# peteroh23/ModulationDetectionCNN

Measured on AMD Instinct MI355X. Metric: I/Q frames/sec (2x128, VT-CNN2, batch=2^20), higher is better.
Workload: dtype bf16; 1 GPU; vtcnn2-c11-bf16-n2^20; topology=vtcnn2, classes=11, frames_per_gpu=1048576, global_batch=1048576, parallelism=batch-shard x1 (no collective), outputs=softmax probabilities f32 + argmax int32, frames_per_forward_call=1048576, full=False

## Files before the change

modulationdetectioncnn_amd/csrc/mdc_api.hip:

```cpp
#include "mdc_internal.h"

#include <cstdlib>
#include <cstring>
#include <exception>
#include <mutex>
#include <new>

namespace mdc {

static thread_local char g_err[512] = "";

void set_error(const char* fmt, ...) {
    va_list ap;
    va_start(ap, fmt);
    vsnprintf(g_err, sizeof(g_err), fmt, ap);
    va_end(ap);
}

int upload(mdc_model* m, int idx, const void* host, size_t bytes) {
    if (m->d_pack[idx]) {
        (void)hipFree(m->d_pack[idx]);
        m->d_pack[idx] = nullptr;
    }
    MDC_HIP(hipMalloc(&m->d_pack[idx], bytes));
// ... 28 lines not shown
    if (hop < 1 || hop > (int64_t)1 << 24) { set_error("%s: hop must be in 1..2^24 sample pairs (got %lld)", who, (long long)hop); return MDC_EINVAL; }
    if (!(level > 0.f) || !(level <= 3.402823466e38f)) { set_error("%s: level must be finite and > 0", who); return MDC_EINVAL; }
    if ((flags & ~MDC_IQ_REMOVE_DC) != 0) { set_error("%s: unknown flag bits 0x%x", who, flags & ~MDC_IQ_REMOVE_DC); return MDC_EINVAL; }
    return MDC_OK;
}

}

using namespace mdc;

static int layer_layout(mdc_model* m) {
    const mdc_topology& t = m->topo;
    switch (t.kind) {
        case MDC_KIND_DEPLOYED:
            if (t.filters != 3 && t.filters != 10) { set_error("deployed: filters must be 3 or 10 (got %d)", t.filters); return MDC_ENOTSUP; }
            if (t.classes != 3) { set_error("deployed: classes must be 3 (got %d)", t.classes); return MDC_ENOTSUP; }
            m->nlayers = 2;
            m->nk[0] = 2 * (size_t)t.filters;            m->nb[0] = t.filters;
            m->nk[1] = 258 * (size_t)t.filters * t.classes; m->nb[1] = t.classes;
            m->slots = {{"mdc_deployed_fwd"}};
            return MDC_OK;
        case MDC_KIND_VTCNN2:
            if (t.classes < 2 || t.classes > 16) { set_error("vtcnn2: classes must be in 2..16 (got %d)", t.classes); return MDC_ENOTSUP; }
            m->nlayers = 4;
            m->nk[0] = (size_t)kC1 * 3;               m->nb[0] = kC1;
            m->nk[1] = (size_t)kC2 * kC1 * 2 * 3;     m->nb[1] = kC2;
            m->nk[2] = (size_t)kFeat * kHid;          m->nb[2] = kHid;
            m->nk[3] = (size_t)kHid * t.classes;      m->nb[3] = t.classes;
            m->slots = {{"mdc_vt_conv"}, {"mdc_vt_dense1"}, {"mdc_vt_head"}};
            return MDC_OK;
        case MDC_KIND_CNNPY:
            if (t.filters < 1 || t.filters > 10 || t.hidden < 1 || t.hidden > 16 || t.classes < 2 || t.classes > 16) {
                set_error("cnnpy: need filters 1..10, hidden 1..16, classes 2..16 (got %d,%d,%d)", t.filters, t.hidden, t.classes);
                return MDC_ENOTSUP;
            }
            m->nlayers = 3;
            m->nk[0] = 2 * 128 * (size_t)t.filters;        m->nb[0] = t.filters;
            m->nk[1] = 3 * (size_t)t.filters * t.hidden;    m->nb[1] = t.hidden;
            m->nk[2] = (size_t)t.hidden * t.classes;        m->nb[2] = t.classes;
            m->slots = {{"mdc_dense_chain"}};
            return MDC_OK;
        default:
            set_error("unknown topology kind %d", t.kind);
            return MDC_EINVAL;
    }
}

extern "C" {

int mdc_abi_version(void) { return MDC_ABI_VERSION; }

const char* mdc_last_error(void) { return g_err; }

int mdc_create(const mdc_topology* topo, int device, mdc_model** out) {
    return guarded("mdc_create", [&]() -> int {
        if (!topo || !out) { set_error("mdc_create: null argument"); return MDC_EINVAL; }
        *out = nullptr;
        if ((topo->reserved[0] & ~MDC_OPT_ALL) != 0) { set_error("mdc_create: unknown option bits 0x%x in reserved[0]", topo->reserved[0]); return MDC_EINVAL; }
        for (int i = 1; i < 4; ++i) if (topo->reserved[i] != 0) { set_error("mdc_create: reserved[1..3] must be 0"); return MDC_EINVAL; }
        if ((topo->reserved[0] & MDC_OPT_FP8_BF16_FEATURES) && topo->kind != MDC_KIND_VTCNN2) {
            set_error("mdc_create: MDC_OPT_FP8_BF16_FEATURES applies to MDC_KIND_VTCNN2 only");
            return MDC_EINVAL;
        }
        int ndev = 0;
        if (hipGetDeviceCount(&ndev) != hipSuccess || ndev == 0) { set_error("no HIP device available"); return MDC_ENODEV; }
        if (device < 0 || device >= ndev) { set_error("device %d out of range (have %d)", device, ndev); return MDC_ENODEV; }
        hipDeviceProp_t prop;
        MDC_HIP(hipGetDeviceProperties(&prop, device));
        if (std::strncmp(prop.gcnArchName, "gfx950", 6) != 0) {
            set_error("device %d is %s; libmdc.so carries gfx950 (MI355X) code only", device, prop.gcnArchName);
            return MDC_ENODEV;
        }
        mdc_model* m = new (std::nothrow) mdc_model();
        if (!m) { set_error("out of host memory"); return MDC_ENOMEM; }
        m->topo = *topo;
        m->device = device;
#ifdef MDC_ALTERNATES
        {
            auto flag = [](const char* name, int when) { const char* e = getenv(name); return e && atoi(e) == when; };
            if (flag("MDC_CONV_SCHED", 0)) m->alt |= kAltConvHipcc;
            if (flag("MDC_DENSE1_PHASED", 0)) m->alt |= kAltDense1Simple;
            if (flag("MDC_DEP_F32_MFMA", 1)) m->alt |= kAltDepF32Mfma;
            if (flag("MDC_D1_FUSED_HEAD", 0)) m->alt |= kAltSeparateHead;
            if (const char* e = getenv("MDC_DEP_RING")) m->alt_ring = atoi(e);
        }
#endif
        int rc = MDC_ENOMEM;
        try { rc = layer_layout(m); } catch (...) { delete m; throw; }
        if (rc != MDC_OK) { delete m; return rc; }
        *out = m;
        return MDC_OK;
    });
}

int mdc_num_layers(const mdc_model* m) {
    if (!m) { set_error("null model"); return MDC_EINVAL; }
    return m->nlayers;
}

int mdc_layer_sizes(const mdc_model* m, int layer, size_t* kernel_elems, size_t* bias_elems) {
    if (!m || layer < 0 || layer >= m->nlayers) { set_error("mdc_layer_sizes: bad layer %d", layer); return MDC_EINVAL; }
    if (kernel_elems) *kernel_elems = m->nk[layer];
    if (bias_elems) *bias_elems = m->nb[layer];
    return MDC_OK;
}

int mdc_set_weights(mdc_model* m, int layer, const float* kernel_host, size_t kernel_elems,
                    const float* bias_host, size_t bias_elems) {
    return guarded("mdc_set_weights", [&]() -> int {
        if (!m || !kernel_host || !bias_host) { set_error("mdc_set_weights: null argument"); return MDC_EINVAL; }
        if (m->finalized) { set_error("mdc_set_weights: model is finalized (immutable)"); return MDC_ESTATE; }
        if (layer < 0 || layer >= m->nlayers) { set_error("mdc_set_weights: layer %d out of range 0..%d", layer, m->nlayers - 1); return MDC_EINVAL; }
        if (kernel_elems != m->nk[layer] || bias_elems != m->nb[layer]) {
            set_error("mdc_set_weights: layer %d expects kernel %zu / bias %zu elements, got %zu / %zu",
                      layer, m->nk[layer], m->nb[layer], kernel_elems, bias_elems);
            return MDC_EINVAL;
        }
        m->have[layer] = false;
        m->hk[layer].assign(kernel_host, kernel_host + kernel_elems);
        m->hb[layer].assign(bias_host, bias_host + bias_elems);
        m->have[layer] = true;
        return MDC_OK;
    });
}

int mdc_finalize(mdc_model* m, int dtype) {
    return guarded("mdc_finalize", [&]() -> int {
        if (!m) { set_error("null model"); return MDC_EINVAL; }
        if (m->finalized) { set_error("mdc_finalize: already finalized"); return MDC_ESTATE; }
        for (int l = 0; l < m->nlayers; ++l)
            if (!m->have[l]) { set_error("mdc_finalize: layer %d has no weights", l); return MDC_ESTATE; }
        if (dtype != MDC_F32 && dtype != MDC_BF16 && dtype != MDC_FP8 && dtype != MDC_F16) { set_error("unknown dtype %d", dtype); return MDC_EINVAL; }
        if (dtype == MDC_F16 && m->topo.kind != MDC_KIND_DEPLOYED) { set_error("f16 is implemented for the deployed nets only"); return MDC_ENOTSUP; }
        if (dtype == MDC_FP8 && m->topo.kind == MDC_KIND_CNNPY) { set_error("fp8 is implemented for the vtcnn2 and deployed families only"); return MDC_ENOTSUP; }
        if ((m->topo.reserved[0] & MDC_OPT_FP8_BF16_FEATURES) && dtype != MDC_FP8) { set_error("mdc_finalize: MDC_OPT_FP8_BF16_FEATURES is an option of the MDC_FP8 mode"); return MDC_EINVAL; }
        if (dtype == MDC_BF16 && m->topo.kind == MDC_KIND_CNNPY) { set_error("bf16 is implemented for the vtcnn2 and deployed families only"); return MDC_ENOTSUP; }
        m->dtype = dtype;
        DeviceScope dev(m->device);
        if (!dev.ok) { set_error("mdc_finalize: cannot select device %d", m->device); return MDC_EIO; }
        int rc;
        switch (m->topo.kind) {
            case MDC_KIND_DEPLOYED:
                rc = deployed_pack(m);
                if (rc == MDC_OK) rc = deployed_q612_pack(m);
                if (rc == MDC_OK && dtype != MDC_F32) rc = deployed_bf16_pack(m);
                break;
            case MDC_KIND_VTCNN2:   rc = vtcnn2_pack(m); break;
            case MDC_KIND_CNNPY:    rc = cnnpy_pack(m); break;
            default: rc = MDC_EINVAL;
        }
        if (rc != MDC_OK) return rc;
        for (int l = 0; l < m->nlayers; ++l) {
            std::vector<float>().swap(m->hk[l]);
            std::vector<float>().swap(m->hb[l]);
        }
        m->finalized = true;
        return MDC_OK;
    });
}

size_t mdc_workspace_bytes(const mdc_model* m, int64_t n) {
    if (!m || n <= 0) return 0;
    if (m->topo.kind == MDC_KIND_VTCNN2) return vtcnn2_workspace_bytes(m, n);
    return 0;
}

// ... 273 lines not shown
```

modulationdetectioncnn_amd/csrc/mdc_internal.h:

```cpp
#pragma once
#include <hip/hip_runtime.h>
#include <cstdarg>
#include <cstdint>
#include <cstdio>
#include <exception>
#include <mutex>
#include <new>
#include <string>
#include <type_traits>
#include <vector>

#include "mdc.h"

namespace mdc {

void set_error(const char* fmt, ...);

template <class Fn>
inline int guarded(const char* what, Fn&& fn) noexcept {
    try {
        return fn();
    } catch (const std::bad_alloc&) {
        set_error("%s: out of host memory", what);
        return MDC_ENOMEM;
    } catch (const std::exception& e) {
        set_error("%s: %s", what, e.what());
        return MDC_EIO;
    } catch (...) {
        set_error("%s: unexpected exception", what);
        return MDC_EIO;
    }
}

#define MDC_HIP(call)                                                                      \
    do {                                                                                   \
        hipError_t e_ = (call);                                                            \
        if (e_ != hipSuccess) {                                                            \
            mdc::set_error("%s failed: %s (%s:%d)", #call, hipGetErrorString(e_), __FILE__, __LINE__); \
            return MDC_EIO;                                                                \
        }                                                                                  \
    } while (0)

constexpr int kRows = 2;
constexpr int kSamples = 128;
constexpr int kFrameFloats = kRows * kSamples;

constexpr int kC1 = 256;
constexpr int kW1 = 130;
constexpr int kC2 = 80;
constexpr int kW2 = 132;
constexpr int kFeat = kC2 * kW2;
constexpr int kHid = 256;

__host__ __device__ constexpr int feat16_index(int w, int o) {
    return (w >> 1) * (2 * kC2) + (o < 64 ? (w & 1) * 64 + o : 128 + 2 * (o - 64) + (w & 1));
}

__host__ __device__ constexpr int feat8_index(int w, int o) {
    return (w >> 2) * (4 * kC2) + (o < 64 ? ((w >> 1) & 1) * 128 + 8 * (o >> 2) + 4 * (w & 1) + (o & 3) : 256 + 4 * (o - 64) + (w & 3));
}

__device__ __forceinline__ uint2 load8_unaligned(const unsigned char* p) {
    uint2 r;
    __builtin_memcpy(&r, p, 8);
    return r;
}

struct NfArgs {
    unsigned char* flags;
    unsigned long long* count;
    int poison;
};
template <bool CHECK> using HopOrNf = typename std::conditional<CHECK, NfArgs, long>::type;
__device__ __forceinline__ long hop_of(long h) { return h; }
__device__ __forceinline__ long hop_of(const NfArgs&) { return 256; }
__device__ __forceinline__ NfArgs nf_of(long) { return NfArgs{nullptr, nullptr, 0}; }
__device__ __forceinline__ NfArgs nf_of(const NfArgs& a) { return a; }
constexpr unsigned kNfInfBits = 0x7F800000u;
__device__ __forceinline__ unsigned nf_absbits_max4(const float4 v) {
    return max(max(__float_as_uint(v.x) & 0x7FFFFFFFu, __float_as_uint(v.y) & 0x7FFFFFFFu),
               max(__float_as_uint(v.z) & 0x7FFFFFFFu, __float_as_uint(v.w) & 0x7FFFFFFFu));
}

enum { kAltConvHipcc = 1,
       kAltDense1Simple = 2,
       kAltDepF32Mfma = 4,
       kAltSeparateHead = 8 };

struct ProfSlot {
    const char* name;
    std::vector<hipEvent_t> ev;
    double total_ms = 0;
    int64_t launches = 0;
};

}

struct mdc_model {
    mdc_topology topo{};
    int device = 0;
    int dtype = MDC_F32;
    bool finalized = false;
    int nlayers = 0;
    size_t nk[4]{}, nb[4]{};
    std::vector<float> hk[4], hb[4];
    bool have[4]{};

    void* d_pack[8]{};
    size_t pack_bytes[8]{};

    int alt = 0;
    int alt_ring = -1;
    float fp8_input_absmax = 0.02f;
    float fp8_feature_absmax = 0.f;
    int fp8_feat_scale_log2 = 0;
    bool fp8_e4m3_features = false;
    float fp8_feat_divisor = 1.f;
    int feat_scale_log2 = 0;

    bool profiling = false;
    std::vector<mdc::ProfSlot> slots;
    std::mutex prof_mu;

    void* host_ctx = nullptr;
    std::mutex host_mu;
};

namespace mdc {

struct ProfScope {
    mdc_model* m;
    int slot;
    hipStream_t s;
    hipEvent_t start = nullptr;
    ProfScope(const mdc_model* mm, int slot_, hipStream_t s_);
    ~ProfScope();
    ProfScope(const ProfScope&) = delete;
    ProfScope& operator=(const ProfScope&) = delete;
};

int upload(mdc_model* m, int idx, const void* host, size_t bytes);

struct DeviceScope {
    int prev = -1, want;
    bool ok = true;
    explicit DeviceScope(int device) : want(device) {
        if (hipGetDevice(&prev) != hipSuccess) prev = -1;
        if (prev != want && hipSetDevice(want) != hipSuccess) ok = false;
    }
    ~DeviceScope() { if (prev >= 0 && prev != want) (void)hipSetDevice(prev); }
    DeviceScope(const DeviceScope&) = delete;
    DeviceScope& operator=(const DeviceScope&) = delete;
};

int predict_host(mdc_model* m, const float* x_host, int64_t n, float* probs_host, int32_t* labels_host, int64_t chunk_frames);
int predict_host_checked(mdc_model* m, const float* x_host, int64_t n, float* probs_host, int32_t* labels_host, uint8_t* nonfinite_host,
                         int64_t* nonfinite_count, int policy, int64_t chunk_frames);
int predict_host_iq_u8(mdc_model* m, const uint8_t* iq_host, int64_t n, int64_t hop, float scale, float* probs_host, int32_t* labels_host,
                       int64_t chunk_frames);
int predict_host_iq_u8_norm(mdc_model* m, const uint8_t* iq_host, int64_t n, int64_t hop, float level, int flags, float* probs_host,
                            int32_t* labels_host, mdc_iq_window_stats* stats_host, int64_t chunk_frames);
int predict_host_iq(mdc_model* m, const void* iq_host, int format, int64_t n, int64_t hop, float scale, float* probs_host, int32_t* labels_host,
                    int64_t chunk_frames);
int predict_host_iq_norm(mdc_model* m, const void* iq_host, int format, int64_t n, int64_t hop, float level, int flags, float* probs_host,
                         int32_t* labels_host, mdc_iq_window_stats64* stats_host, int64_t chunk_frames);
void host_ctx_free(mdc_model* m);

int deployed_pack(mdc_model* m);
int deployed_f32m_pack(mdc_model* m);
int deployed_f32m_forward(const mdc_model* m, const float* x, int64_t n, float* probs, int32_t* labels, float* tap_dense, hipStream_t s);
// ... 42 lines not shown
```

modulationdetectioncnn_amd/csrc/vtcnn2_bf16_dense1.hip:

```cpp
#include "vtcnn2_bf16_common.h"
#include "dense_chain_common.h"

#include <cstdlib>

namespace mdc {

namespace {

constexpr int kBM = 256, kBN = 256, kBK = 64;
constexpr int kTileBytes = kBM * kBK * 2;
constexpr size_t kDenseBf16Lds = (size_t)4 * kTileBytes;
constexpr size_t kDenseHeadLds = (size_t)128 * kChainXld * 4;
static_assert(kDenseHeadLds >= kDenseBf16Lds, "the fused-head form allocates the larger of the two");
constexpr int kNT = kFeat / kBK;

__device__ __forceinline__ bf16x8 cvt_e4m3x8(u32x2 r) {
    const bf16x2 p0 = __builtin_amdgcn_cvt_scalef32_pk_bf16_fp8(r[0], 1.0f, false);
    const bf16x2 p1 = __builtin_amdgcn_cvt_scalef32_pk_bf16_fp8(r[0], 1.0f, true);
    const bf16x2 p2 = __builtin_amdgcn_cvt_scalef32_pk_bf16_fp8(r[1], 1.0f, false);
    const bf16x2 p3 = __builtin_amdgcn_cvt_scalef32_pk_bf16_fp8(r[1], 1.0f, true);
    return bf16x8{p0[0], p0[1], p1[0], p1[1], p2[0], p2[1], p3[0], p3[1]};
}


// ... 67 lines not shown
                for (int j = 0; j < 4; ++j)
                    acc[i][j] = __builtin_amdgcn_mfma_f32_16x16x32_bf16(af[i], bfr[j], acc[i][j], 0, 0, 0);
        }
    };

    stage(0, 0);
    __syncthreads();
    int cur = 0;
    for (int t = 0; t < kNT - 1; ++t) {
        stage(t + 1, cur ^ 1);
        compute(cur);
        __syncthreads();
        cur ^= 1;
    }
    compute(cur);

#pragma unroll
    for (int j = 0; j < 4; ++j) {
        const int col = wc * 64 + j * 16 + fr;
        const float bias = c1[col];
#pragma unroll
        for (int i = 0; i < 8; ++i)
#pragma unroll
            for (int r = 0; r < 4; ++r) {
                const long row = row0 + wr * 128 + i * 16 + fg * 4 + r;
                if (row < n) hid[row * kHid + col] = fmaxf(acc[i][j][r] + bias, 0.f);
            }
    }
}


#endif

template <bool HEAD>
__device__ __forceinline__ void d1_epilogue(f32x4 (&acc)[8][4], unsigned char* smem, long row0, long n, int lane, int wv,
                                            const float* __restrict__ c1, float* __restrict__ hid, const float* __restrict__ w2pack,
                                            int n_out, float* __restrict__ probs, int* __restrict__ labels) {
    const int wr = wv >> 2, wc = wv & 3, fr = lane & 15, fg = lane >> 4;
    if constexpr (!HEAD) {
#pragma unroll
        for (int j = 0; j < 4; ++j) {
            const int col = wc * 64 + j * 16 + fr;
            const float bias = c1[col];
#pragma unroll
            for (int i = 0; i < 8; ++i)
#pragma unroll
                for (int r = 0; r < 4; ++r) {
                    const long row = row0 + wr * 128 + i * 16 + fg * 4 + r;
                    if (row < n) hid[row * kHid + col] = fmaxf(acc[i][j][r] + bias, 0.f);
                }
        }
    } else {
        float* xs = reinterpret_cast<float*>(smem);
        float w2[64];
#pragma unroll
        for (int i = 0; i < 64; ++i) w2[i] = w2pack[i * 64 + lane];
        const float b2 = w2pack[64 * 64 + 16 * 64 + fr];
        float bias1[4];
#pragma unroll
        for (int j = 0; j < 4; ++j) bias1[j] = c1[wc * 64 + j * 16 + fr];
#pragma unroll
        for (int half = 0; half < 2; ++half) {
            __syncthreads();
            if (wr == half) {
#pragma unroll
                for (int j = 0; j < 4; ++j)
#pragma unroll
                    for (int i = 0; i < 8; ++i)
#pragma unroll
                        for (int r = 0; r < 4; ++r)
                            xs[(i * 16 + fg * 4 + r) * kChainXld + wc * 64 + j * 16 + fr] = fmaxf(acc[i][j][r] + bias1[j], 0.f);
            }
            __syncthreads();
            const f32x4 a2 = chain_k256(xs + (wv * 16 + fr) * kChainXld + fg, w2, f32x4{0.f, 0.f, 0.f, 0.f});
            f32x4 z;
#pragma unroll
            for (int r = 0; r < 4; ++r) z[r] = a2[r] + b2;
            chain_softmax_store(z, fr, fg, row0 + half * 128 + wv * 16, n, n_out, probs, labels, nullptr);
        }
    }
}

constexpr int kUnitBytes = 128 * 128;

template <int ABL, bool HEAD = false, bool F8 = false>
__global__ __launch_bounds__(512) void vt_dense1_bf16_phased_kernel(const unsigned short* __restrict__ feat, long n,
                                                                    const unsigned short* __restrict__ w1t,
                                                                    const float* __restrict__ c1, float* __restrict__ hid,
                                                                    const float* __restrict__ w2pack = nullptr, int n_out = 0,
                                                                    float* __restrict__ probs = nullptr, int* __restrict__ labels = nullptr) {
    extern __shared__ __attribute__((aligned(16))) unsigned char smem[];
    const int tid = threadIdx.x, lane = tid & 63;
    const int wv = __builtin_amdgcn_readfirstlane(tid >> 6);
    const int wr = wv >> 2, wc = wv & 3;
    const int fr = lane & 15, fg = lane >> 4;
    const long row0 = (long)blockIdx.x * kBM;

    const int srow = lane >> 3, spos = lane & 7;
    const unsigned short* src[4][2];
#pragma unroll
    for (int j = 0; j < 2; ++j) {
        const int u = (wv * 2 + j) * 8 + srow;
        const int sw = (spos ^ (u & 7)) * 8;
        const int arow_lo = 128 * (u >> 6) + (u & 63);
        const int brow_lo = 64 * (u >> 5) + (u & 31);
        long g0 = (ABL == 1 ? 0 : row0) + arow_lo, g3 = (ABL == 1 ? 0 : row0) + arow_lo + 64;
        if (g0 >= n) g0 = n - 1;
        if (g3 >= n) g3 = n - 1;
        src[0][j] = feat + g0 * (long)kFeat + sw;
        src[3][j] = feat + g3 * (long)kFeat + sw;
        src[1][j] = w1t + brow_lo * kBK + sw;
        src[2][j] = w1t + (brow_lo + 32) * kBK + sw;
    }
    const unsigned char* src8[2] = {nullptr, nullptr};
    if constexpr (F8) {
        const int u = wv * 16 + (lane >> 2);
        const int sw = ((lane & 3) ^ ((u >> 2) & 3)) * 16;
        const int arow_lo = 128 * (u >> 6) + (u & 63);
        long g0 = row0 + arow_lo, g3 = row0 + arow_lo + 64;
        if (g0 >= n) g0 = n - 1;
        if (g3 >= n) g3 = n - 1;
        const unsigned char* f8 = reinterpret_cast<const unsigned char*>(feat);
        src8[0] = f8 + g0 * (long)kFeat + sw;
        src8[1] = f8 + g3 * (long)kFeat + sw;
    }
    auto stage_unit = [&](int t, int unit, int b) {
        if (ABL == 2 && (unit == 1 || unit == 2) && (t & 1)) return;
        unsigned char* dst = smem + ((size_t)b * 4 + unit) * kUnitBytes + (wv * 2) * 1024;
        if constexpr (F8) {
            if (unit == 0 || unit == 3) {
                glds16(src8[unit == 3] + (long)t * kBK, smem + ((size_t)b * 4 + unit) * kUnitBytes + wv * 1024);
                return;
            }
        }
        if (unit == 0 || unit == 3) {
            glds16_nt(src[unit][0] + (long)t * kBK, dst);
            glds16_nt(src[unit][1] + (long)t * kBK, dst + 1024);
        } else {
            glds16(src[unit][0] + (long)t * (kBN * kBK), dst);
            glds16(src[unit][1] + (long)t * (kBN * kBK), dst + 1024);
        }
    };

    auto frag = [&](const unsigned char* unit_base, int u, int ks) {
        return *reinterpret_cast<const bf16x8*>(unit_base + u * 128 + (((ks * 4 + fg) ^ (u & 7)) * 16));
    };

    f32x4 acc[8][4];
#pragma unroll
    for (int i = 0; i < 8; ++i)
#pragma unroll
        for (int j = 0; j < 4; ++j) acc[i][j] = f32x4{0.f, 0.f, 0.f, 0.f};
    bf16x8 a0[4][2], a1[4][2], b0[2][2], b1[2][2];
    u32x2 ra[4][2];

    unsigned ra_lane[2] = {0u, 0u};
    if constexpr (F8) {
        ra_lane[0] = (unsigned)((64 * wr + fr) * 64 + ((((fg >> 1) ^ ((fr >> 2) & 3)) * 16) + (fg & 1) * 8));
        ra_lane[1] = ra_lane[0] ^ 32u;
    }
    auto read_a = [&](bf16x8 (&a)[4][2], int unit, int b) {
        if (ABL == 3 && b == 1) return;
        const unsigned char* base = smem + ((size_t)b * 4 + unit) * kUnitBytes;
        if constexpr (F8) {
            const unsigned bl = (unsigned)(size_t)(__attribute__((address_space(3))) unsigned char*)const_cast<unsigned char*>(base);
            const unsigned ad0 = bl + ra_lane[0], ad1 = bl + ra_lane[1];
#pragma unroll
            for (int i = 0; i < 4; ++i) {
                asm volatile("ds_read_b64 %0, %1 offset:%2" : "=v"(ra[i][0]) : "v"(ad0), "i"(i * 1024) : "memory");
                asm volatile("ds_read_b64 %0, %1 offset:%2" : "=v"(ra[i][1]) : "v"(ad1), "i"(i * 1024) : "memory");
            }
        } else {
#pragma unroll
            for (int i = 0; i < 4; ++i)
#pragma unroll
                for (int ks = 0; ks < 2; ++ks) a[i][ks] = frag(base, 64 * wr + 16 * i + fr, ks);
        }
    };
    auto cvt_a = [&](bf16x8 (&a)[4][2]) {
        if constexpr (F8) {
#pragma unroll
            for (int i = 0; i < 4; ++i)
#pragma unroll
                for (int ks = 0; ks < 2; ++ks) a[i][ks] = cvt_e4m3x8(ra[i][ks]);
        }
    };
    auto read_b = [&](bf16x8 (&bq)[2][2], int unit, int b) {
        if (ABL == 3 && b == 1) return;
        const unsigned char* base = smem + ((size_t)b * 4 + unit) * kUnitBytes;
#pragma unroll
        for (int j = 0; j < 2; ++j)
#pragma unroll
            for (int ks = 0; ks < 2; ++ks) bq[j][ks] = frag(base, 32 * wc + 16 * j + fr, ks);
    };
    auto quadrant = [&](const bf16x8 (&a)[4][2], const bf16x8 (&bq)[2][2], int i0, int j0) {
#ifndef D1_NOPRIO
        __builtin_amdgcn_s_setprio(1);
#endif
#pragma unroll
        for (int ks = 0; ks < 2; ++ks)
#pragma unroll
            for (int i = 0; i < 4; ++i)
#pragma unroll
                for (int j = 0; j < 2; ++j)
                    acc[i0 + i][j0 + j] = __builtin_amdgcn_mfma_f32_16x16x32_bf16(a[i][ks], bq[j][ks], acc[i0 + i][j0 + j], 0, 0, 0);
#ifndef D1_NOPRIO
        __builtin_amdgcn_s_setprio(0);
#endif
    };
    auto quadrant_cv = [&](bf16x8 (&a)[4][2], const bf16x8 (&bq)[2][2], int i0, int j0, bf16x8 (&dst)[4][2], auto own) {
        constexpr bool OWN = decltype(own)::value;
        __builtin_amdgcn_s_setprio(1);
        if constexpr (OWN) a[0][0] = cvt_e4m3x8(ra[0][0]);
#pragma unroll
        for (int f = 0; f < 8; ++f) {
            const int ks = f >> 2, i = f & 3;
            if constexpr (OWN) { if (f + 1 < 8) a[(f + 1) & 3][(f + 1) >> 2] = cvt_e4m3x8(ra[(f + 1) & 3][(f + 1) >> 2]); }
            else dst[i][ks] = cvt_e4m3x8(ra[i][ks]);
#pragma unroll
            for (int j = 0; j < 2; ++j)
                acc[i0 + i][j0 + j] = __builtin_amdgcn_mfma_f32_16x16x32_bf16(a[i][ks], bq[j][ks], acc[i0 + i][j0 + j], 0, 0, 0);
        }
        if constexpr (OWN) __builtin_amdgcn_sched_group_barrier(0x002, 4, 0);
#pragma unroll
        for (int f = 0; f < 16; ++f) {
            __builtin_amdgcn_sched_group_barrier(0x008, 1, 0);
            __builtin_amdgcn_sched_group_barrier(0x002, 2, 0);
        }
        __builtin_amdgcn_s_setprio(0);
    };
#define D1_WAIT_BARRIER(N) do { asm volatile("s_waitcnt vmcnt(" #N ")" ::: "memory"); __builtin_amdgcn_s_barrier(); } while (0)
#define D1_LGKM() asm volatile("s_waitcnt lgkmcnt(0)" ::: "memory")
#define D1_LGKM_RA() asm volatile("s_waitcnt lgkmcnt(0)" : "+v"(ra[0][0]), "+v"(ra[0][1]), "+v"(ra[1][0]), "+v"(ra[1][1]), \
                                  "+v"(ra[2][0]), "+v"(ra[2][1]), "+v"(ra[3][0]), "+v"(ra[3][1]) :: "memory")

#pragma unroll
    for (int u = 0; u < 4; ++u) stage_unit(0, u, 0);
    D1_WAIT_BARRIER(0);
    read_a(a0, 0, 0);
    if constexpr (F8) { D1_LGKM_RA(); cvt_a(a0); }
#ifndef D1_NOSTAGGER
    if (wr == 1) __builtin_amdgcn_s_barrier();
#endif

    for (int t = 0; t < kNT; ++t) {
        const int b = t & 1;
        const bool more = t + 1 < kNT;
        if (more) stage_unit(t + 1, 0, b ^ 1);
        __builtin_amdgcn_sched_barrier(0);
        read_b(b0, 1, b);
        if constexpr (F8) { if (more) D1_WAIT_BARRIER(2); else D1_WAIT_BARRIER(1); }
        else { if (more) D1_WAIT_BARRIER(4); else D1_WAIT_BARRIER(2); }
        D1_LGKM();
        quadrant(a0, b0, 0, 0);
        __builtin_amdgcn_s_barrier();
        if (more) stage_unit(t + 1, 1, b ^ 1);
        __builtin_amdgcn_sched_barrier(0);
        read_b(b1, 2, b);
        if constexpr (F8) { if (more) D1_WAIT_BARRIER(3); else D1_WAIT_BARRIER(0); }
        else { if (more) D1_WAIT_BARRIER(4); else D1_WAIT_BARRIER(0); }
        D1_LGKM();
        quadrant(a0, b1, 0, 2);
        __builtin_amdgcn_s_barrier();
        if (more) stage_unit(t + 1, 2, b ^ 1);
        __builtin_amdgcn_sched_barrier(0);
        read_a(a1, 3, b);
        if (more) D1_WAIT_BARRIER(4); else __builtin_amdgcn_s_barrier();
        if constexpr (F8) { D1_LGKM_RA(); quadrant_cv(a1, b1, 4, 2, a1, std::true_type{}); }
        else { D1_LGKM(); quadrant(a1, b1, 4, 2); }
        __builtin_amdgcn_s_barrier();
        if (more) stage_unit(t + 1, 3, b ^ 1);
        __builtin_amdgcn_sched_barrier(0);
        if (more) read_a(a0, 0, b ^ 1);
        if constexpr (F8) { if (more) D1_WAIT_BARRIER(3); else __builtin_amdgcn_s_barrier(); }
        else { if (more) D1_WAIT_BARRIER(4); else __builtin_amdgcn_s_barrier(); }
        if constexpr (F8) {
            if (more) { D1_LGKM_RA(); quadrant_cv(a1, b0, 4, 0, a0, std::false_type{}); }
            else { D1_LGKM(); quadrant(a1, b0, 4, 0); }
        } else {
            quadrant(a1, b0, 4, 0);
            D1_LGKM();
        }
        __builtin_amdgcn_s_barrier();
    }
#ifndef D1_NOSTAGGER
    if (wr == 0) __builtin_amdgcn_s_barrier();
#endif
#undef D1_WAIT_BARRIER
#undef D1_LGKM
#undef D1_LGKM_RA

    d1_epilogue<HEAD>(acc, smem, row0, n, lane, wv, c1, hid, w2pack, n_out, probs, labels);
}


template <bool F8>
__global__ __launch_bounds__(64) void vt_dense1_bf16_small_kernel(const unsigned short* __restrict__ feat, long n,
                                                                  const unsigned short* __restrict__ w1t,
                                                                  const float* __restrict__ c1, float* __restrict__ hid) {
    const int lane = threadIdx.x, fr = lane & 15, fg = lane >> 4;
    const long row0 = (long)blockIdx.x * 16;
    const int col0 = blockIdx.y * 16;
    long ar = row0 + fr;
    if (ar >= n) ar = n - 1;
    using AFrag = typename std::conditional<F8, u32x2, bf16x8>::type;
    const unsigned char* ap = reinterpret_cast<const unsigned char*>(feat) + (ar * (long)kFeat + fg * 8) * (F8 ? 1 : 2);
    const unsigned short* bp = w1t + (long)(col0 + fr) * kBK + fg * 8;
    f32x4 acc = f32x4{0.f, 0.f, 0.f, 0.f};
    constexpr int kU = 5, kBlocks = kNT / kU;
    static_assert(kNT % kU == 0 && kBlocks % 2 == 1, "blocks: an even count in the loop, the last one drained after it");
    AFrag a0[kU][2], a1[kU][2];
    bf16x8 b0[kU][2], b1[kU][2];
    auto load = [&](AFrag (&af)[kU][2], bf16x8 (&bfr)[kU][2], int blk) {
#pragma unroll
        for (int u = 0; u < kU; ++u)
#pragma unroll
            for (int ks = 0; ks < 2; ++ks) {
                af[u][ks] = *reinterpret_cast<const AFrag*>(ap + ((blk * kU + u) * kBK + ks * 32) * (F8 ? 1 : 2));
                bfr[u][ks] = *reinterpret_cast<const bf16x8*>(bp + (long)(blk * kU + u) * (kBN * kBK) + ks * 32);
            }
    };
    auto mma = [&](const AFrag (&af)[kU][2], const bf16x8 (&bfr)[kU][2]) {
#pragma unroll
        for (int u = 0; u < kU; ++u)
#pragma unroll
            for (int ks = 0; ks < 2; ++ks) {
                bf16x8 a;
                if constexpr (F8) a = cvt_e4m3x8(af[u][ks]); else a = af[u][ks];
                acc = __builtin_amdgcn_mfma_f32_16x16x32_bf16(a, bfr[u][ks], acc, 0, 0, 0);
            }
    };
    load(a0, b0, 0);
    for (int blk = 0; blk < kBlocks - 1; blk += 2) {
        load(a1, b1, blk + 1);
        mma(a0, b0);
        load(a0, b0, blk + 2);
        mma(a1, b1);
    }
    mma(a0, b0);
    const int col = col0 + fr;
    const float bias = c1[col];
#pragma unroll
    for (int r = 0; r < 4; ++r) {
        const long row = row0 + fg * 4 + r;
        if (row < n) hid[row * kHid + col] = fmaxf(acc[r] + bias, 0.f);
    }
}

constexpr int kRing = 24;
constexpr int kGrp = 4;
constexpr size_t kCoopLds = (size_t)kRing * 4096;

template <bool F8>
__global__ __launch_bounds__(256) void vt_dense1_bf16_coop_kernel(const unsigned short* __restrict__ feat, long n,
                                                                  const unsigned short* __restrict__ w1t,
                                                                  const float* __restrict__ c1, float* __restrict__ hid) {
    extern __shared__ __attribute__((aligned(16))) unsigned char smem[];
    const int tid = threadIdx.x, lane = tid & 63, fr = lane & 15, fg = lane >> 4;
    const int wv = __builtin_amdgcn_readfirstlane(tid >> 6);
    const long row0 = (long)blockIdx.x * 16;
    const int col0 = blockIdx.y * 16;
    long ar = row0 + fr;
    if (ar >= n) ar = n - 1;
    const unsigned char* src;
    long kstep;
    if (wv < 2) {
        if constexpr (F8) { src = reinterpret_cast<const unsigned char*>(feat) + ar * (long)kFeat + fg * 16; kstep = kBK; }
        else { src = reinterpret_cast<const unsigned char*>(feat + ar * (long)kFeat + fg * 8 + (wv & 1) * 32); kstep = 2L * kBK; }
    } else {
        src = reinterpret_cast<const unsigned char*>(w1t + (long)(col0 + fr) * kBK + fg * 8 + (wv & 1) * 32);
        kstep = 2L * kBN * kBK;
    }
    const bool copies = !(F8 && wv == 1);
    static_assert(kRing % kGrp == 0, "groups do not straddle the ring's end");
    constexpr int kAhead = kRing / kGrp - 1;
// ... 51 lines not shown
    for (int g = 0; g < kGroups - 1; g += 2) {
        step(f0, f1, g);
        step(f1, f0, g + 1);
    }
    step(f0, f1, kGroups - 1);
    mma(f1, kTail);
    asm volatile("s_waitcnt vmcnt(0)" ::: "memory");
    if (wv != 0) return;
    const int col = col0 + fr;
    const float bias = c1[col];
#pragma unroll
    for (int r = 0; r < 4; ++r) {
        const long row = row0 + fg * 4 + r;
        if (row < n) hid[row * kHid + col] = fmaxf(acc[r] + bias, 0.f);
    }
}

constexpr long kCoopBatch = 256;

constexpr long kSmallBatch = 2048;

}

int vtcnn2_bf16_dense1(const mdc_model* m, const void* feat, int64_t n, float* hid, hipStream_t s,
                       bool fuse_head, float* probs, int32_t* labels, bool* fused) {
    if (fused) *fused = false;
    const bool f8 = m->dtype == MDC_FP8 && m->fp8_e4m3_features;
    if (n <= kCoopBatch) {
#define MDC_LAUNCH_COOP(F) do { \
        MDC_HIP(hipFuncSetAttribute(reinterpret_cast<const void*>(vt_dense1_bf16_coop_kernel<F>), hipFuncAttributeMaxDynamicSharedMemorySize, (int)kCoopLds)); \
        hipLaunchKernelGGL(vt_dense1_bf16_coop_kernel<F>, dim3((unsigned)((n + 15) / 16), kHid / 16), dim3(256), kCoopLds, s, \
                           static_cast<const unsigned short*>(feat), (long)n, static_cast<const unsigned short*>(m->d_pack[3]), \
                           static_cast<const float*>(m->d_pack[4]), hid); } while (0)
        if (f8) MDC_LAUNCH_COOP(true); else MDC_LAUNCH_COOP(false);
#undef MDC_LAUNCH_COOP
        MDC_HIP(hipGetLastError());
        return MDC_OK;
    }
    if (n <= kSmallBatch) {
#define MDC_LAUNCH_SMALL(F) hipLaunchKernelGGL(vt_dense1_bf16_small_kernel<F>, dim3((unsigned)((n + 15) / 16), kHid / 16), dim3(64), 0, s, \
                           static_cast<const unsigned short*>(feat), (long)n, static_cast<const unsigned short*>(m->d_pack[3]), \
                           static_cast<const float*>(m->d_pack[4]), hid)
        if (f8) MDC_LAUNCH_SMALL(true); else MDC_LAUNCH_SMALL(false);
#undef MDC_LAUNCH_SMALL
        MDC_HIP(hipGetLastError());
        return MDC_OK;
    }
    const unsigned short* f = static_cast<const unsigned short*>(feat);
    const unsigned short* w1t = static_cast<const unsigned short*>(m->d_pack[3]);
    const float* c1 = static_cast<const float*>(m->d_pack[4]);
    const dim3 grid((unsigned)((n + kBM - 1) / kBM));
#if defined(MDC_ALTERNATES) || defined(MDC_ABLATIONS)
#define MDC_LAUNCH_D1(A) do { \
    MDC_HIP(hipFuncSetAttribute(reinterpret_cast<const void*>(vt_dense1_bf16_kernel<A>), hipFuncAttributeMaxDynamicSharedMemorySize, (int)kDenseBf16Lds)); \
    hipLaunchKernelGGL(vt_dense1_bf16_kernel<A>, grid, dim3(512), kDenseBf16Lds, s, f, (long)n, w1t, c1, hid); } while (0)
#endif
#ifdef MDC_ABLATIONS
    static const int abl = getenv("MDC_ABLATE_D1") ? atoi(getenv("MDC_ABLATE_D1")) : 0;
#define MDC_LAUNCH_PROBE(A) do { \
        MDC_HIP(hipFuncSetAttribute(reinterpret_cast<const void*>(vt_dense1_bf16_phased_kernel<A>), hipFuncAttributeMaxDynamicSharedMemorySize, (int)kDenseBf16Lds)); \
        hipLaunchKernelGGL(vt_dense1_bf16_phased_kernel<A>, grid, dim3(512), kDenseBf16Lds, s, f, (long)n, w1t, c1, hid); \
        MDC_HIP(hipGetLastError()); \
        return MDC_OK; } while (0)
    if (!f8 && abl == 10) MDC_LAUNCH_PROBE(0);
    if (!f8 && abl == 11) MDC_LAUNCH_PROBE(1);
    if (!f8 && abl == 12) MDC_LAUNCH_PROBE(2);
    if (!f8 && abl == 13) MDC_LAUNCH_PROBE(3);
#undef MDC_LAUNCH_PROBE
    if (abl >= 1 && abl <= 3) {
        switch (abl) { case 1: MDC_LAUNCH_D1(1); break; case 2: MDC_LAUNCH_D1(2); break; default: MDC_LAUNCH_D1(3); }
        MDC_HIP(hipGetLastError());
        return MDC_OK;
    }
#endif
#ifdef MDC_ALTERNATES
    if (!f8 && (m->alt & kAltDense1Simple)) {
        MDC_LAUNCH_D1(0);
        MDC_HIP(hipGetLastError());
        return MDC_OK;
    }
    if (m->alt & kAltSeparateHead) fuse_head = false;
#endif
#undef MDC_LAUNCH_D1
#define MDC_LAUNCH_PHASED(F) do { \
    if (fuse_head && (probs || labels)) { \
        MDC_HIP(hipFuncSetAttribute(reinterpret_cast<const void*>(vt_dense1_bf16_phased_kernel<0, true, F>), hipFuncAttributeMaxDynamicSharedMemorySize, (int)kDenseHeadLds)); \
        hipLaunchKernelGGL((vt_dense1_bf16_phased_kernel<0, true, F>), grid, dim3(512), kDenseHeadLds, s, f, (long)n, w1t, c1, hid, \
                           static_cast<const float*>(m->d_pack[5]), (int)m->topo.classes, probs, labels); \
        if (fused) *fused = true; \
    } else { \
        MDC_HIP(hipFuncSetAttribute(reinterpret_cast<const void*>(vt_dense1_bf16_phased_kernel<0, false, F>), hipFuncAttributeMaxDynamicSharedMemorySize, (int)kDenseBf16Lds)); \
        hipLaunchKernelGGL((vt_dense1_bf16_phased_kernel<0, false, F>), grid, dim3(512), kDenseBf16Lds, s, f, (long)n, w1t, c1, hid); \
    } } while (0)
    if (f8) MDC_LAUNCH_PHASED(true); else MDC_LAUNCH_PHASED(false);
#undef MDC_LAUNCH_PHASED
    MDC_HIP(hipGetLastError());
    return MDC_OK;
}

}
```

Before: 41.45 million frames/s.

## Restructure bf16 dense1 K-loop into two-quadrant windows with earlier staging

Adds a WIN=4 variant of the phased dense1 GEMM kernel, now the default for bf16 features. Each K-step runs as two windows of two quadrants each instead of the previous schedule, and the A tile for step t+2 is prefetched one step ahead. Global-to-LDS loads use inline asm with a scalar base plus precomputed 32-bit offsets instead of per-unit pointer arrays, which saves VGPRs and address arithmetic. The intent is to hide load latency behind MFMAs with fewer barriers and waits. The cost is a hand-tuned waitcnt schedule that is fragile if load counts change, and the old 8-window path stays available behind an env flag.

```diff
diff --git a/modulationdetectioncnn_amd/csrc/mdc_api.hip b/modulationdetectioncnn_amd/csrc/mdc_api.hip
--- a/modulationdetectioncnn_amd/csrc/mdc_api.hip
+++ b/modulationdetectioncnn_amd/csrc/mdc_api.hip
@@ -134,6 +134,7 @@
             if (flag("MDC_DENSE1_PHASED", 0)) m->alt |= kAltDense1Simple;
             if (flag("MDC_DEP_F32_MFMA", 1)) m->alt |= kAltDepF32Mfma;
             if (flag("MDC_D1_FUSED_HEAD", 0)) m->alt |= kAltSeparateHead;
+            if (flag("MDC_DENSE1_WINDOWS", 8)) m->alt |= kAltDense1Win8;
             if (const char* e = getenv("MDC_DEP_RING")) m->alt_ring = atoi(e);
         }
 #endif
diff --git a/modulationdetectioncnn_amd/csrc/mdc_internal.h b/modulationdetectioncnn_amd/csrc/mdc_internal.h
--- a/modulationdetectioncnn_amd/csrc/mdc_internal.h
+++ b/modulationdetectioncnn_amd/csrc/mdc_internal.h
@@ -85,7 +85,8 @@
 enum { kAltConvHipcc = 1,
        kAltDense1Simple = 2,
        kAltDepF32Mfma = 4,
-       kAltSeparateHead = 8 };
+       kAltSeparateHead = 8,
+       kAltDense1Win8 = 16 };
 
 struct ProfSlot {
     const char* name;
diff --git a/modulationdetectioncnn_amd/csrc/vtcnn2_bf16_dense1.hip b/modulationdetectioncnn_amd/csrc/vtcnn2_bf16_dense1.hip
--- a/modulationdetectioncnn_amd/csrc/vtcnn2_bf16_dense1.hip
+++ b/modulationdetectioncnn_amd/csrc/vtcnn2_bf16_dense1.hip
@@ -173,13 +173,18 @@
 }
 
 constexpr int kUnitBytes = 128 * 128;
-
-template <int ABL, bool HEAD = false, bool F8 = false>
+#ifndef MDC_D1_WINDOWS
+#define MDC_D1_WINDOWS 4
+#endif
+constexpr int kDense1Windows = MDC_D1_WINDOWS;
+
+template <int ABL, bool HEAD = false, bool F8 = false, int WIN = 8>
 __global__ __launch_bounds__(512) void vt_dense1_bf16_phased_kernel(const unsigned short* __restrict__ feat, long n,
                                                                     const unsigned short* __restrict__ w1t,
                                                                     const float* __restrict__ c1, float* __restrict__ hid,
                                                                     const float* __restrict__ w2pack = nullptr, int n_out = 0,
                                                                     float* __restrict__ probs = nullptr, int* __restrict__ labels = nullptr) {
+    static_assert(WIN == 8 || (WIN == 4 && ABL == 0 && !F8), "two-quadrant windows: the bf16-feature product form only");
     extern __shared__ __attribute__((aligned(16))) unsigned char smem[];
     const int tid = threadIdx.x, lane = tid & 63;
     const int wv = __builtin_amdgcn_readfirstlane(tid >> 6);
@@ -189,8 +194,26 @@
 
     const int srow = lane >> 3, spos = lane & 7;
     const unsigned short* src[4][2];
+    unsigned aoff[2][2] = {{0u, 0u}, {0u, 0u}}, boff = 0u;
+    const unsigned char* const abase = reinterpret_cast<const unsigned char*>(feat + row0 * (long)kFeat);
+    if constexpr (WIN == 4) {
+#pragma unroll
+        for (int j = 0; j < 2; ++j) {
+            const int u = (wv * 2 + j) * 8 + srow;
+            const int sw = (spos ^ (u & 7)) * 8;
+            const int arow_lo = 128 * (u >> 6) + (u & 63);
+            long g0 = row0 + arow_lo, g3 = row0 + arow_lo + 64;
+            if (g0 >= n) g0 = n - 1;
+            if (g3 >= n) g3 = n - 1;
+            aoff[0][j] = (unsigned)((g0 - row0) * kFeat + sw) * 2u;
+            aoff[1][j] = (unsigned)((g3 - row0) * kFeat + sw) * 2u;
+        }
+        const int u = wv * 16 + srow;
+        boff = (unsigned)((64 * (u >> 5) + (u & 31)) * kBK + (spos ^ (u & 7)) * 8) * 2u;
+    }
 #pragma unroll
     for (int j = 0; j < 2; ++j) {
+        if constexpr (WIN == 4) break;
         const int u = (wv * 2 + j) * 8 + srow;
         const int sw = (spos ^ (u & 7)) * 8;
         const int arow_lo = 128 * (u >> 6) + (u & 63);
@@ -224,6 +247,19 @@
                 return;
             }
         }
+        if constexpr (WIN == 4) {
+            const unsigned l = (unsigned)(size_t)(__attribute__((address_space(3))) unsigned char*)dst;
+            if (unit == 0 || unit == 3) {
+                const unsigned char* base = abase + (long)t * (kBK * 2);
+                asm volatile("global_load_lds_dwordx4 %0, %1 nt" ::"v"(aoff[unit == 3][0]), "s"(base), "{m0}"(l) : "memory");
+                asm volatile("global_load_lds_dwordx4 %0, %1 nt" ::"v"(aoff[unit == 3][1]), "s"(base), "{m0}"(l + 1024u) : "memory");
+            } else {
+                const unsigned char* base = reinterpret_cast<const unsigned char*>(w1t) + (long)t * (kBN * kBK * 2) + (unit == 2 ? 32 * kBK * 2 : 0);
+                asm volatile("global_load_lds_dwordx4 %0, %1" ::"v"(boff), "s"(base), "{m0}"(l) : "memory");
+                asm volatile("global_load_lds_dwordx4 %0, %1" ::"v"(boff), "s"(base + 8 * kBK * 2), "{m0}"(l + 1024u) : "memory");
+            }
+            return;
+        }
         if (unit == 0 || unit == 3) {
             glds16_nt(src[unit][0] + (long)t * kBK, dst);
             glds16_nt(src[unit][1] + (long)t * kBK, dst + 1024);
@@ -299,6 +335,15 @@
         __builtin_amdgcn_s_setprio(0);
 #endif
     };
+    auto quadrant_np = [&](const bf16x8 (&a)[4][2], const bf16x8 (&bq)[2][2], int i0, int j0) {
+#pragma unroll
+        for (int ks = 0; ks < 2; ++ks)
+#pragma unroll
+            for (int i = 0; i < 4; ++i)
+#pragma unroll
+                for (int j = 0; j < 2; ++j)
+                    acc[i0 + i][j0 + j] = __builtin_amdgcn_mfma_f32_16x16x32_bf16(a[i][ks], bq[j][ks], acc[i0 + i][j0 + j], 0, 0, 0);
+    };
     auto quadrant_cv = [&](bf16x8 (&a)[4][2], const bf16x8 (&bq)[2][2], int i0, int j0, bf16x8 (&dst)[4][2], auto own) {
         constexpr bool OWN = decltype(own)::value;
         __builtin_amdgcn_s_setprio(1);
@@ -327,13 +372,52 @@
 
 #pragma unroll
     for (int u = 0; u < 4; ++u) stage_unit(0, u, 0);
-    D1_WAIT_BARRIER(0);
+    if constexpr (WIN == 4) {
+        static_assert(kNT >= 2, "the prologue stages a unit of tile 1");
+        stage_unit(1, 0, 1);
+        D1_WAIT_BARRIER(4);
+    } else {
+        D1_WAIT_BARRIER(0);
+    }
     read_a(a0, 0, 0);
     if constexpr (F8) { D1_LGKM_RA(); cvt_a(a0); }
+    if constexpr (WIN == 4) D1_LGKM();
 #ifndef D1_NOSTAGGER
     if (wr == 1) __builtin_amdgcn_s_barrier();
 #endif
 
+    if constexpr (WIN == 4) {
+    for (int t = 0; t < kNT; ++t) {
+        const int b = t & 1;
+        const bool more = t + 1 < kNT, more2 = t + 2 < kNT;
+        if (more) { stage_unit(t + 1, 1, b ^ 1); stage_unit(t + 1, 2, b ^ 1); }
+        __builtin_amdgcn_sched_barrier(0);
+        read_b(b0, 1, b);
+        read_b(b1, 2, b);
+        if (more) D1_WAIT_BARRIER(4); else D1_WAIT_BARRIER(0);
+        D1_LGKM();
+        __builtin_amdgcn_s_setprio(1);
+        quadrant_np(a0, b0, 0, 0);
+        quadrant_np(a0, b1, 0, 2);
+        __builtin_amdgcn_s_setprio(0);
+        __builtin_amdgcn_s_barrier();
+        if (more) stage_unit(t + 1, 3, b ^ 1);
+        if (more2) stage_unit(t + 2, 0, b);
+        __builtin_amdgcn_sched_barrier(0);
+        read_a(a1, 3, b);
+        __builtin_amdgcn_sched_barrier(0);
+        if (more) read_a(a0, 0, b ^ 1);
+        if (more2) D1_WAIT_BARRIER(4); else if (more) D1_WAIT_BARRIER(2); else __builtin_amdgcn_s_barrier();
+        if (more) asm volatile("s_waitcnt lgkmcnt(8)" ::: "memory");
+        else D1_LGKM();
+        __builtin_amdgcn_s_setprio(1);
+        quadrant_np(a1, b1, 4, 2);
+        quadrant_np(a1, b0, 4, 0);
+        __builtin_amdgcn_s_setprio(0);
+        D1_LGKM();
+        __builtin_amdgcn_s_barrier();
+    }
+    } else
     for (int t = 0; t < kNT; ++t) {
         const int b = t & 1;
         const bool more = t + 1 < kNT;
@@ -381,7 +465,13 @@
 #undef D1_LGKM
 #undef D1_LGKM_RA
 
-    d1_epilogue<HEAD>(acc, smem, row0, n, lane, wv, c1, hid, w2pack, n_out, probs, labels);
+    if constexpr (WIN == 4) {
+        int lane_e;
+        asm volatile("v_mbcnt_lo_u32_b32 %0, -1, 0\n\tv_mbcnt_hi_u32_b32 %0, -1, %0" : "=v"(lane_e));
+        d1_epilogue<HEAD>(acc, smem, row0, n, lane_e, wv, c1, hid, w2pack, n_out, probs, labels);
+    } else {
+        d1_epilogue<HEAD>(acc, smem, row0, n, lane, wv, c1, hid, w2pack, n_out, probs, labels);
+    }
 }
 
 
@@ -599,17 +689,21 @@
     if (m->alt & kAltSeparateHead) fuse_head = false;
 #endif
 #undef MDC_LAUNCH_D1
-#define MDC_LAUNCH_PHASED(F) do { \
+#define MDC_LAUNCH_PHASED(F, W) do { \
     if (fuse_head && (probs || labels)) { \
-        MDC_HIP(hipFuncSetAttribute(reinterpret_cast<const void*>(vt_dense1_bf16_phased_kernel<0, true, F>), hipFuncAttributeMaxDynamicSharedMemorySize, (int)kDenseHeadLds)); \
-        hipLaunchKernelGGL((vt_dense1_bf16_phased_kernel<0, true, F>), grid, dim3(512), kDenseHeadLds, s, f, (long)n, w1t, c1, hid, \
+        MDC_HIP(hipFuncSetAttribute(reinterpret_cast<const void*>(vt_dense1_bf16_phased_kernel<0, true, F, W>), hipFuncAttributeMaxDynamicSharedMemorySize, (int)kDenseHeadLds)); \
+        hipLaunchKernelGGL((vt_dense1_bf16_phased_kernel<0, true, F, W>), grid, dim3(512), kDenseHeadLds, s, f, (long)n, w1t, c1, hid, \
                            static_cast<const float*>(m->d_pack[5]), (int)m->topo.classes, probs, labels); \
         if (fused) *fused = true; \
     } else { \
-        MDC_HIP(hipFuncSetAttribute(reinterpret_cast<const void*>(vt_dense1_bf16_phased_kernel<0, false, F>), hipFuncAttributeMaxDynamicSharedMemorySize, (int)kDenseBf16Lds)); \
-        hipLaunchKernelGGL((vt_dense1_bf16_phased_kernel<0, false, F>), grid, dim3(512), kDenseBf16Lds, s, f, (long)n, w1t, c1, hid); \
+        MDC_HIP(hipFuncSetAttribute(reinterpret_cast<const void*>(vt_dense1_bf16_phased_kernel<0, false, F, W>), hipFuncAttributeMaxDynamicSharedMemorySize, (int)kDenseBf16Lds)); \
+        hipLaunchKernelGGL((vt_dense1_bf16_phased_kernel<0, false, F, W>), grid, dim3(512), kDenseBf16Lds, s, f, (long)n, w1t, c1, hid); \
     } } while (0)
-    if (f8) MDC_LAUNCH_PHASED(true); else MDC_LAUNCH_PHASED(false);
+    if (f8) MDC_LAUNCH_PHASED(true, 8);
+#ifdef MDC_ALTERNATES
+    else if (m->alt & kAltDense1Win8) MDC_LAUNCH_PHASED(false, 8);
+#endif
+    else MDC_LAUNCH_PHASED(false, kDense1Windows);
 #undef MDC_LAUNCH_PHASED
     MDC_HIP(hipGetLastError());
     return MDC_OK;
```

After: 41.56 million frames/s (median of 6 runs). Within noise of the previous version (+0.3%).
